# sailfish-team/sailfish

Measured on AMD Instinct MI355X. Metric: MLUPS (million lattice updates/s), D3Q19 BGK 512^3 per GPU, higher is better.
Workload: dtype f32; 1 GPU; D3Q19 BGK periodic box, 512x512x512 nodes per GPU, global 512x512x512 (fluid nodes only counted); access_pattern=AB, periodic=in-sweep wrap, decomposition=single subdomain, block_x=512, repeats=1

## Files before the change

sailfish_amd/csrc/slf_api.hip:

```cpp
#include <hip/hip_runtime.h>
#include <dlfcn.h>
#include <stdio.h>
#include <string.h>

#include <algorithm>
#include <string>
#include <vector>

#include "../../include/sailfish_hip.h"
#include "slf_kernels.h"
#include "slf_node.h"

#ifndef SLF_DEFAULT_VARIANT
#define SLF_DEFAULT_VARIANT 11
#endif

namespace {

thread_local std::string g_last_error;

int fail(int code, const std::string& msg) {
  g_last_error = msg;
  return code;
}

int hip_fail(hipError_t e, const char* what) {
  return fail(SLF_ERR_HIP, std::string(what) + ": " + hipGetErrorString(e));
}

#define SLF_HIP(call)                            \
  do {                                           \
    hipError_t _e = (call);                      \
    if (_e != hipSuccess) return hip_fail(_e, #call); \
  } while (0)

enum KernelKind {
  KK_COLLIDE_AND_PROPAGATE,
  KK_SET_INITIAL_CONDITIONS,
  KK_PBC,
  KK_PBC_SWAP,
  KK_MACRO_PBC,
  KK_COLLECT_SPARSE,
  KK_DISTRIBUTE_SPARSE,
  KK_COLLECT_BOX,
  KK_DISTRIBUTE_BOX,
  KK_COLLECT_FACE_SWAP,
  KK_DISTRIBUTE_FACE_SWAP,
  KK_COLLECT_MACRO_FACE,
  KK_DISTRIBUTE_MACRO_FACE,
  KK_COMPUTE_MACRO,
  KK_SC_MACRO,
  KK_SC_SWEEP0,
  KK_SC_SWEEP1,
  KK_SC_FUSED,
  KK_SC_INIT,
  KK_SCS_MACRO,
  KK_SCS_SWEEP,
  KK_RESIDENT,
};

}

struct slf_ctx {
  int device;
};
struct slf_stream {
  slf_ctx* ctx;
  hipStream_t s;
};
struct slf_event {
  slf_ctx* ctx;
  hipEvent_t e;
};
struct slf_graph {
  hipGraph_t graph;
  hipGraphExec_t exec;
};
struct slf_module {
  slf_ctx* ctx;
  slf::KernelSelector sel;
  slf::Geometry geo;
  slf::Physics phys;
  slf::ShanChen sc;
  int access_pattern;
  int block_x;
  void* node_params;
  uint32_t* status;
  void* xsend[2];
  void* xrecv[2];
  void* sc_send[3][2];
  void* sc_recv[3][2];
  slf::RowClasses rows;
  void* rows_mem;
  slf::SlotTable slots;
  void* slots_mem;
  int n_node_params, precision;
  void* stage[4];
  hipEvent_t stage_ev[4];
  size_t stage_bytes[4];
  int stage_next;
};
struct slf_kernel {
  slf_module* mod;
  KernelKind kind;
  std::vector<unsigned long long> ptrs;
  std::vector<long long> ints;
  int needs_iteration;
  uint32_t iteration;
  bool bound;
  bool sc_local_velocity;
  bool alpha_arg = false;
  int pair_rows = 0, pair_zc = 0;
  int pair_prefetch = 0;
};

static hipStream_t native(slf_stream* s) { return s ? s->s : (hipStream_t)0; }

static const slf::SlotTable* slot_table_for(slf_module* m, const void* nodes, hipStream_t s) {
  static const bool enabled = [] { const char* v = getenv("SLF_INDIRECT_SLOTS"); return !(v && atoi(v) == 0); }();
  if (!enabled || !nodes || !m->geo.indirect) return nullptr;
  if (m->slots.nodes == nodes) return &m->slots;
  if (m->geo.lat_ny > 65535 || m->geo.lat_nz > 65535) return nullptr;
  if (m->slots_mem) {
    hipFree(m->slots_mem);
    m->slots_mem = nullptr;
  }
  m->slots = slf::SlotTable{};
  const size_t n = m->geo.dist_size;
  char* mem = nullptr;
  if (hipMalloc((void**)&mem, 2 * n * sizeof(uint32_t) + 256) != hipSuccess) return nullptr;
  uint32_t* max_slot = (uint32_t*)(mem + 2 * n * sizeof(uint32_t));
  uint32_t h = 0;
  hipError_t e = hipMemsetAsync(mem, 0xFF, 2 * n * sizeof(uint32_t), s);
  if (e == hipSuccess) e = hipMemsetAsync(max_slot, 0, 256, s);
  if (e == hipSuccess) e = slf::launch_build_slot_table(m->geo, nodes, (uint32_t*)mem, (uint32_t*)mem + n, max_slot, s);
  if (e == hipSuccess) e = hipMemcpyAsync(&h, max_slot, sizeof(h), hipMemcpyDeviceToHost, s);
  if (e == hipSuccess) e = hipStreamSynchronize(s);
  if (e != hipSuccess) {
    hipFree(mem);
    return nullptr;
  }
  m->slots_mem = mem;
  m->slots.nodes = nodes;
  m->slots.slot_gi = (const uint32_t*)mem;
  m->slots.slot_yz = (const uint32_t*)mem + n;
  m->slots.n_slots = h + 1;
  return &m->slots;
}

extern "C" {

int slf_abi_version(void) { return SLF_ABI_VERSION; }

const char* slf_last_error(void) { return g_last_error.c_str(); }

int slf_device_count(int* count) {
  if (!count) return fail(SLF_ERR_INVALID, "count is NULL");
  hipError_t e = hipGetDeviceCount(count);
  if (e != hipSuccess) {
    *count = 0;
    return hip_fail(e, "hipGetDeviceCount");
  }
  return SLF_OK;
}

int slf_device_pci_bus_id(int device, char* out, size_t len) {
  if (!out || len < 13) return fail(SLF_ERR_INVALID, "buffer of at least 13 bytes needed");
  SLF_HIP(hipDeviceGetPCIBusId(out, (int)len, device));
  return SLF_OK;
}

int slf_ctx_create(int device, slf_ctx** out) {
  if (!out) return fail(SLF_ERR_INVALID, "out is NULL");
  int n = 0;
  SLF_HIP(hipGetDeviceCount(&n));
  if (device < 0 || device >= n) return fail(SLF_ERR_INVALID, "no such HIP device");
  SLF_HIP(hipSetDevice(device));
  slf_ctx* c = new slf_ctx;
  c->device = device;
  *out = c;
  return SLF_OK;
}

int slf_ctx_destroy(slf_ctx* ctx) {
  delete ctx;
  return SLF_OK;
}

int slf_ctx_sync(slf_ctx* ctx) {
  if (!ctx) return fail(SLF_ERR_INVALID, "ctx is NULL");
  SLF_HIP(hipSetDevice(ctx->device));
  SLF_HIP(hipDeviceSynchronize());
  return SLF_OK;
}

int slf_ctx_info(slf_ctx* ctx, char* name, size_t name_len, size_t* total_mem, int* cu_count, int* wavefront) {
  if (!ctx) return fail(SLF_ERR_INVALID, "ctx is NULL");
  hipDeviceProp_t prop;
  SLF_HIP(hipGetDeviceProperties(&prop, ctx->device));
  if (name && name_len) {
    snprintf(name, name_len, "%s (%s)", prop.name, prop.gcnArchName);
  }
  if (total_mem) *total_mem = prop.totalGlobalMem;
  if (cu_count) *cu_count = prop.multiProcessorCount;
  if (wavefront) *wavefront = prop.warpSize;
  return SLF_OK;
}

int slf_ctx_free_memory(slf_ctx* ctx, size_t* free_bytes) {
  if (!ctx || !free_bytes) return fail(SLF_ERR_INVALID, "NULL argument");
  SLF_HIP(hipSetDevice(ctx->device));
  size_t total = 0;
  SLF_HIP(hipMemGetInfo(free_bytes, &total));
  return SLF_OK;
}

int slf_malloc(slf_ctx* ctx, size_t bytes, void** dptr) {
  if (!ctx || !dptr) return fail(SLF_ERR_INVALID, "NULL argument");
  SLF_HIP(hipSetDevice(ctx->device));
  SLF_HIP(hipMalloc(dptr, bytes ? bytes : 1));
  return SLF_OK;
}

int slf_free(slf_ctx* ctx, void* dptr) {
  if (!ctx) return fail(SLF_ERR_INVALID, "ctx is NULL");
  if (dptr) SLF_HIP(hipFree(dptr));
  return SLF_OK;
}

int slf_memset(slf_ctx* ctx, void* dptr, int value, size_t bytes, slf_stream* stream) {
  if (!ctx || !dptr) return fail(SLF_ERR_INVALID, "NULL argument");
  SLF_HIP(hipMemsetAsync(dptr, value, bytes, native(stream)));
  if (!stream) SLF_HIP(hipStreamSynchronize(nullptr));
  return SLF_OK;
}

int slf_vmm_granularity(slf_ctx* ctx, size_t* bytes) {
  if (!ctx || !bytes) return fail(SLF_ERR_INVALID, "NULL argument");
  hipMemAllocationProp prop = {};
  prop.type = hipMemAllocationTypePinned;
  prop.location.type = hipMemLocationTypeDevice;
  prop.location.id = ctx->device;
  SLF_HIP(hipMemGetAllocationGranularity(bytes, &prop, hipMemAllocationGranularityRecommended));
  return SLF_OK;
}

int slf_vmm_reserve(slf_ctx* ctx, size_t bytes, void** va) {
  if (!ctx || !va) return fail(SLF_ERR_INVALID, "NULL argument");
  SLF_HIP(hipSetDevice(ctx->device));
  SLF_HIP(hipMemAddressReserve(va, bytes, 0, nullptr, 0));
  return SLF_OK;
}

int slf_vmm_release_range(slf_ctx* ctx, void* va, size_t bytes) {
  if (!ctx) return fail(SLF_ERR_INVALID, "ctx is NULL");
  SLF_HIP(hipMemAddressFree(va, bytes));
  return SLF_OK;
}

int slf_vmm_chunk_create(slf_ctx* ctx, size_t bytes, uint64_t* handle) {
  if (!ctx || !handle) return fail(SLF_ERR_INVALID, "NULL argument");
  SLF_HIP(hipSetDevice(ctx->device));
  hipMemAllocationProp prop = {};
  prop.type = hipMemAllocationTypePinned;
  prop.location.type = hipMemLocationTypeDevice;
  prop.location.id = ctx->device;
// ... 1260 lines not shown
      case 'i': k->ints.push_back(*(const int32_t*)argv[i]); break;
      default: return fail(SLF_ERR_INVALID, std::string("unsupported format char: ") + fmt[i]);
    }
  }
  const int dim = k->mod->geo.dim;
  size_t want_p = 0, want_i = 0;
  switch (k->kind) {
    case KK_COLLIDE_AND_PROPAGATE:
    case KK_COMPUTE_MACRO: want_p = 4 + dim; want_i = 1; break;
    case KK_SET_INITIAL_CONDITIONS: want_p = 3 + dim; want_i = 0; break;
    case KK_PBC:
    case KK_PBC_SWAP:
    case KK_MACRO_PBC: want_p = 1; want_i = 1; break;
    case KK_COLLECT_SPARSE:
    case KK_DISTRIBUTE_SPARSE: want_p = 3; want_i = 1; break;
    case KK_COLLECT_BOX:
    case KK_DISTRIBUTE_BOX:
      want_p = 2;
      want_i = (k->ints.size() == 8) ? 8 : 6;
      if (k->ints.size() == (dim == 3 ? 5u : 3u)) {
        want_i = k->ints.size();
        if (strcmp(fmt, dim == 3 ? "PiiiiiP" : "PiiiP")) return fail(SLF_ERR_INVALID, "reference form: the buffer is the last argument");
        if (k->mod->geo.indirect) return fail(SLF_ERR_UNSUPPORTED, "indirect addressing: halo through index lists");
      }
      break;
    case KK_COLLECT_FACE_SWAP:
    case KK_DISTRIBUTE_FACE_SWAP:
      want_p = 2; want_i = dim == 3 ? 5 : 3;
      if (strcmp(fmt, dim == 3 ? "PiiiiiP" : "PiiiP")) return fail(SLF_ERR_INVALID, "arguments: (dist, face, base_gx[, base_other], max_lx[, max_other], buffer)");
      break;
    case KK_COLLECT_MACRO_FACE:
    case KK_DISTRIBUTE_MACRO_FACE:
      want_p = 2; want_i = dim == 3 ? 5 : 3;
      if (strcmp(fmt, dim == 3 ? "PiiiiiP" : "PiiiP")) return fail(SLF_ERR_INVALID, "arguments: (field, [face,] base_gx, ..., buffer)");
      break;
    case KK_SC_MACRO:
    case KK_SC_SWEEP0:
    case KK_SC_SWEEP1: want_p = 5 + dim; want_i = 1; break;
    case KK_SC_FUSED: want_p = 7 + dim; want_i = 1; break;
    case KK_SC_INIT: want_p = 5 + dim; want_i = 0; break;
    case KK_SCS_MACRO: want_p = 3; want_i = 1; break;
    case KK_SCS_SWEEP: want_p = 4 + dim; want_i = 1; break;
    case KK_RESIDENT: want_p = 5; want_i = 5; break;
  }
  if (k->kind == KK_RESIDENT && k->ptrs.size() == 5 && k->ints.size() == 5) {
    const bool aa = k->mod->access_pattern == SLF_AA;
    const int steps = (int)k->ints[1], tx = (int)k->ints[2], ty = (int)k->ints[3], halo = (int)k->ints[4];
    if (!needs_iteration) return fail(SLF_ERR_INVALID, "CollideAndPropagateResident needs the iteration argument (its first step)");
    if (steps < 1 || tx < 1 || ty < 1 || halo < 1) return fail(SLF_ERR_INVALID, "steps, tile and halo must be positive");
    if (!k->ptrs[1] || !k->ptrs[3] || (!aa && (!k->ptrs[2] || !k->ptrs[4])))
      return fail(SLF_ERR_INVALID, "CollideAndPropagateResident: source and destination arrays (both copies of the two-copy pattern)");
    if (k->ptrs[1] == k->ptrs[3] || (!aa && k->ptrs[2] == k->ptrs[4]))
      return fail(SLF_ERR_INVALID, "CollideAndPropagateResident: source and destination must be different buffers");
    const int need = std::max(slf::resident_halo(aa, 0, steps), slf::resident_halo(aa, 1, steps));
    if (halo < need) return fail(SLF_ERR_INVALID, "CollideAndPropagateResident: halo too small for this many steps");
    const long long nw = (long long)(tx + 2 * halo) * (long long)(ty + 2 * halo);
    if (nw > 2 * 1024) return fail(SLF_ERR_INVALID, "CollideAndPropagateResident: window larger than 2048 nodes");
    const int q = 9;
    if (slf::resident_lds_bytes(q, k->mod->sel.precision, aa, tx + 2 * halo, ty + 2 * halo) + 4352 > 160 * 1024)
      return fail(SLF_ERR_INVALID, "CollideAndPropagateResident: window does not fit the 160 KiB of LDS");
  }
  if (k->mod->geo.indirect && (k->kind == KK_SC_FUSED || k->sc_local_velocity))
    return fail(SLF_ERR_UNSUPPORTED, "indirect addressing: the binary model runs the reference's pass and its two per-lattice sweeps");
  if (k->mod->geo.indirect && (k->kind == KK_COLLIDE_AND_PROPAGATE || k->kind == KK_COMPUTE_MACRO ||
                               k->kind == KK_SET_INITIAL_CONDITIONS || k->kind == KK_SC_MACRO ||
                               k->kind == KK_SC_SWEEP0 || k->kind == KK_SC_SWEEP1 || k->kind == KK_SC_INIT ||
                               k->kind == KK_SCS_MACRO || k->kind == KK_SCS_SWEEP))
    want_p += 1;
  k->alpha_arg = false;
  if (k->kind == KK_COLLIDE_AND_PROPAGATE && k->mod->sel.model == SLF_ELBM && k->ptrs.size() == want_p + 1 &&
      fmt[argc - 1] == 'P') {
    want_p += 1;
    k->alpha_arg = true;
  }
  if (k->ptrs.size() != want_p || k->ints.size() != want_i)
    return fail(SLF_ERR_INVALID, "argument list does not match the kernel's signature");
  k->pair_rows = k->pair_zc = 0;
  k->needs_iteration = needs_iteration;
  k->bound = true;
  if (k->kind == KK_COLLIDE_AND_PROPAGATE && k->mod->geo.indirect && !k->ptrs.empty() &&
      k->mod->phys.incompressible != SLF_DENSITY_ROUNDOFF && !k->mod->phys.regularized && !k->mod->phys.subgrid &&
      k->mod->sel.model != SLF_ELBM) {
    SLF_HIP(hipSetDevice(k->mod->ctx->device));
    slot_table_for(k->mod, (const void*)k->ptrs[0], (hipStream_t)0);
  }
  return SLF_OK;
}

int slf_kernel_set_iteration(slf_kernel* k, uint32_t iteration) {
  if (!k) return fail(SLF_ERR_INVALID, "kernel is NULL");
  k->iteration = iteration;
  return SLF_OK;
}

namespace {


int step_prop(const slf_kernel* k, slf::Prop* prop) {
  *prop = slf::PROP_AB;
  if (k->mod->access_pattern == SLF_AA) {
    if (!k->needs_iteration) return fail(SLF_ERR_INVALID, "AA kernels need the iteration argument");
    *prop = (k->iteration & 1u) ? slf::PROP_AA_ODD : slf::PROP_AA_EVEN;
  }
  return SLF_OK;
}

int sweep_region(const slf::Geometry& g, const slf_region* region, int* y0, int* y1, int* z0, int* z1) {
  *y0 = 1; *y1 = g.lat_ny - 1; *z0 = 1; *z1 = g.lat_nz - 1;
  if (g.dim == 2) { *z0 = 0; *z1 = 1; }
  if (region) {
    *y0 = region->y0; *y1 = region->y1;
    if (g.dim == 3) { *z0 = region->z0; *z1 = region->z1; }
    if (*y0 < 1 || *y1 > g.lat_ny - 1 || *y0 > *y1 || (g.dim == 3 && (*z0 < 1 || *z1 > g.lat_nz - 1 || *z0 > *z1)))
      return fail(SLF_ERR_INVALID, "region outside the real nodes of the subdomain");
  }
  return SLF_OK;
}

int sweep_common(const slf_kernel* k, slf::SweepArgs& a) {
  a.node_params = k->mod->node_params;
  a.status = k->mod->status;
  a.options = (uint32_t)k->ints[0];
  if (k->mod->sel.general && !a.map) return fail(SLF_ERR_INVALID, "node map is NULL but the module is not fluid_only");
  return SLF_OK;
}

void pair_args(const slf_kernel* k, slf::SweepArgs& a) {
  const slf_module* m = k->mod;
  const int b0 = m->geo.indirect ? 1 : 0;
  a.nodes = m->geo.indirect ? (const void*)k->ptrs[0] : nullptr;
  a.map = (const void*)k->ptrs[b0 + 0];
  a.dist_in = (void*)k->ptrs[b0 + 1];
  a.dist_out = (void*)k->ptrs[b0 + 2];
  a.node_params = m->node_params;
  a.status = m->status;
  a.options = (uint32_t)k->ints[0];
  for (int f = 0; f < 2; f++) {
    a.xsend[f] = m->xsend[f];
    a.xrecv[f] = m->xrecv[f];
  }
}

}

int slf_kernel_set_pair(slf_kernel* k, int rows_per_strip, int planes_per_chunk) {
  if (!k) return fail(SLF_ERR_INVALID, "kernel is NULL");
  if (k->kind != KK_COLLIDE_AND_PROPAGATE)
    return fail(SLF_ERR_UNSUPPORTED, "pair sweep: CollideAndPropagate kernels of single-fluid modules only");
  if (!k->bound) return fail(SLF_ERR_INVALID, "pair sweep: set the kernel arguments first (source and destination are checked)");
  if (rows_per_strip < 0 || planes_per_chunk < 0) return fail(SLF_ERR_INVALID, "pair sweep: negative strip / chunk size");
  const slf_module* m = k->mod;
  const int rows = rows_per_strip ? rows_per_strip : slf::pair_default_rows(m->geo);
  const int zc = planes_per_chunk ? planes_per_chunk : slf::pair_default_zchunk(m->geo);
  int prefetch = slf::pair_default_prefetch();
  if (const char* e = getenv("SLF_PAIR_PREFETCH")) {
    char* end = nullptr;
    const long v = strtol(e, &end, 10);
    if (*e) prefetch = (end && !*end && v >= 0 && v < 1000) ? (int)v : -1;
  }
  if (m->sc.enabled || m->sel.lattice != SLF_D3Q19 || k->alpha_arg)
    return fail(SLF_ERR_UNSUPPORTED, "pair sweep: D3Q19, single precision, BGK modules only");
  slf::SweepArgs a = {};
  pair_args(k, a);
  if (const char* why = slf::pair_refusal(m->sel, m->access_pattern == SLF_AB, m->geo, m->phys, a, rows, zc, prefetch))
    return fail(SLF_ERR_UNSUPPORTED, why);
  k->pair_rows = rows;
  k->pair_zc = zc;
  k->pair_prefetch = prefetch;
  return SLF_OK;
}

int slf_kernel_launch(slf_kernel* k, const slf_region* region, slf_stream* stream) {
  if (!k) return fail(SLF_ERR_INVALID, "kernel is NULL");
  if (!k->bound) return fail(SLF_ERR_INVALID, "kernel arguments not set");
  slf_module* m = k->mod;
  const slf::Geometry& g = m->geo;
  SLF_HIP(hipSetDevice(m->ctx->device));
  hipStream_t s = native(stream);
  hipError_t e = hipSuccess;
  switch (k->kind) {
    case KK_COLLIDE_AND_PROPAGATE:
    case KK_COMPUTE_MACRO: {
      if (k->pair_rows) {
        slf::SweepArgs pa = {};
        pair_args(k, pa);
        if (region) return fail(SLF_ERR_UNSUPPORTED, "pair sweep: whole-box launches only");
        if (!slf::launch_sweep_pair(m->sel, m->access_pattern == SLF_AB, g, m->phys, pa, k->pair_rows, k->pair_zc, k->pair_prefetch, s,
                                    &e)) {
          const char* why = slf::pair_refusal(m->sel, m->access_pattern == SLF_AB, g, m->phys, pa, k->pair_rows, k->pair_zc,
                                              k->pair_prefetch);
          return fail(SLF_ERR_UNSUPPORTED, why ? why : "pair sweep: no kernel for this strip size");
        }
        break;
      }
      slf::SweepArgs a = {};
      const int b0 = g.indirect ? 1 : 0;
      a.nodes = g.indirect ? (const void*)k->ptrs[0] : nullptr;
      a.map = (const void*)k->ptrs[b0 + 0];
      a.dist_in = (void*)k->ptrs[b0 + 1];
      a.dist_out = (void*)k->ptrs[b0 + 2];
      a.rho = (void*)k->ptrs[b0 + 3];
      a.phi = nullptr;
      a.v[0] = (void*)k->ptrs[b0 + 4];
      a.v[1] = (void*)k->ptrs[b0 + 5];
      a.v[2] = g.dim == 3 ? (void*)k->ptrs[b0 + 6] : nullptr;
      a.alpha = k->alpha_arg ? (void*)k->ptrs.back() : nullptr;
      for (int f = 0; f < 2; f++) {
        a.xsend[f] = m->xsend[f];
        a.xrecv[f] = m->xrecv[f];
      }
      a.rows = m->rows.map ? &m->rows : nullptr;
      if (int rc = sweep_common(k, a)) return rc;
      if (g.indirect && !a.nodes) return fail(SLF_ERR_INVALID, "indirect addressing: the nodes table is NULL");
      if (g.indirect && k->kind == KK_COLLIDE_AND_PROPAGATE && m->slots.nodes == a.nodes) a.slots = &m->slots;
      slf::Prop prop;
      if (int rc = step_prop(k, &prop)) return rc;
      if (k->kind == KK_COMPUTE_MACRO) {
        e = slf::launch_macro(m->sel, prop, g, m->phys, a, s);
        break;
      }
      int y0, y1, z0, z1;
      if (int rc = sweep_region(g, region, &y0, &y1, &z0, &z1)) return rc;
      e = slf::launch_sweep(m->sel, prop, g, m->phys, a, y0, y1, z0, z1, m->block_x, s);
      break;
    }
    case KK_SC_MACRO:
    case KK_SC_SWEEP0:
    case KK_SC_SWEEP1: {
      slf::SweepArgs a = {};
      const int b0 = g.indirect ? 1 : 0;
      a.nodes = g.indirect ? (const void*)k->ptrs[0] : nullptr;
      if (g.indirect && !a.nodes) return fail(SLF_ERR_INVALID, "indirect addressing: the nodes table is NULL");
      a.map = (const void*)k->ptrs[b0 + 0];
      a.dist_in = (void*)k->ptrs[b0 + 1];
      a.dist_out = (void*)k->ptrs[b0 + 2];
      a.rho = (void*)k->ptrs[b0 + 3];
      a.phi = (void*)k->ptrs[b0 + 4];
      a.v[0] = (void*)k->ptrs[b0 + 5];
      a.v[1] = (void*)k->ptrs[b0 + 6];
      a.v[2] = g.dim == 3 ? (void*)k->ptrs[b0 + 7] : nullptr;
      a.sc_local_velocity = k->sc_local_velocity;
      sc_planes_of(m, a);
      if (int rc = sweep_common(k, a)) return rc;
      slf::Prop prop;
      if (int rc = step_prop(k, &prop)) return rc;
      int y0, y1, z0, z1;
      if (int rc = sweep_region(g, region, &y0, &y1, &z0, &z1)) return rc;
      if (k->kind == KK_SC_MACRO) e = slf::launch_sc_macro(m->sel, prop, g, m->phys, m->sc, a, y0, y1, z0, z1, s);
      else e = slf::launch_sc_sweep(m->sel, k->kind == KK_SC_SWEEP0 ? 0 : 1, prop, g, m->phys, m->sc, a, y0, y1, z0, z1,
                                    m->block_x, s);
      break;
    }
    case KK_SC_FUSED: {
      slf::SweepArgs a = {};
      a.map = (const void*)k->ptrs[0];
      a.dist_in = (void*)k->ptrs[1];
      a.dist_out = (void*)k->ptrs[2];
      a.dist_in2 = (void*)k->ptrs[3];
      a.dist_out2 = (void*)k->ptrs[4];
      a.rho = (void*)k->ptrs[5];
      a.phi = (void*)k->ptrs[6];
      a.v[0] = (void*)k->ptrs[7];
      a.v[1] = (void*)k->ptrs[8];
      a.v[2] = g.dim == 3 ? (void*)k->ptrs[9] : nullptr;
      a.sc_local_velocity = k->sc_local_velocity;
      sc_planes_of(m, a);
      if (int rc = sweep_common(k, a)) return rc;
      slf::Prop prop;
      if (int rc = step_prop(k, &prop)) return rc;
      int y0, y1, z0, z1;
      if (int rc = sweep_region(g, region, &y0, &y1, &z0, &z1)) return rc;
      e = slf::launch_sc_fused(m->sel, prop, g, m->phys, m->sc, a, y0, y1, z0, z1, m->block_x, s);
      break;
    }
    case KK_RESIDENT: {
      slf::SweepArgs a = {};
      a.map = (const void*)k->ptrs[0];
      a.node_params = m->node_params;
      a.status = m->status;
      a.options = (uint32_t)k->ints[0] & ~1u;
      if (m->sel.general && !a.map) return fail(SLF_ERR_INVALID, "node map is NULL but the module is not fluid_only");
      const void* src[2] = {(const void*)k->ptrs[1], (const void*)k->ptrs[2]};
      void* dst[2] = {(void*)k->ptrs[3], (void*)k->ptrs[4]};
      e = slf::launch_resident(m->sel, m->access_pattern == SLF_AA, g, m->phys, a, src, dst, (int)k->iteration, (int)k->ints[1],
                               (int)k->ints[2], (int)k->ints[3], (int)k->ints[4], s);
      break;
    }
    case KK_SCS_MACRO:
    case KK_SCS_SWEEP: {
      slf::SweepArgs a = {};
      const int b0 = g.indirect ? 1 : 0;
      a.nodes = g.indirect ? (const void*)k->ptrs[0] : nullptr;
      if (g.indirect && !a.nodes) return fail(SLF_ERR_INVALID, "indirect addressing: the nodes table is NULL");
      a.map = (const void*)k->ptrs[b0 + 0];
      a.dist_in = (void*)k->ptrs[b0 + 1];
      a.phi = nullptr;
      if (k->kind == KK_SCS_MACRO) {
        a.dist_out = nullptr;
        a.rho = (void*)k->ptrs[b0 + 2];
        a.v[0] = a.v[1] = a.v[2] = nullptr;
      } else {
        a.dist_out = (void*)k->ptrs[b0 + 2];
        a.rho = (void*)k->ptrs[b0 + 3];
        a.v[0] = (void*)k->ptrs[b0 + 4];
        a.v[1] = (void*)k->ptrs[b0 + 5];
        a.v[2] = g.dim == 3 ? (void*)k->ptrs[b0 + 6] : nullptr;
      }
      sc_planes_of(m, a);
      if (int rc = sweep_common(k, a)) return rc;
      slf::Prop prop;
      if (int rc = step_prop(k, &prop)) return rc;
      if (k->kind == KK_SCS_MACRO) {
        e = slf::launch_scs_macro(m->sel, prop, g, m->phys, m->sc, a, s);
        break;
      }
      int y0, y1, z0, z1;
      if (int rc = sweep_region(g, region, &y0, &y1, &z0, &z1)) return rc;
      e = slf::launch_scs_sweep(m->sel, prop, g, m->phys, m->sc, a, y0, y1, z0, z1, m->block_x, s);
      break;
    }
    case KK_SC_INIT: {
      const int b0 = g.indirect ? 1 : 0;
      if (g.indirect && !k->ptrs[0]) return fail(SLF_ERR_INVALID, "indirect addressing: the nodes table is NULL");
      const void* v[3] = {(const void*)k->ptrs[b0 + 3], (const void*)k->ptrs[b0 + 4],
                          g.dim == 3 ? (const void*)k->ptrs[b0 + 5] : nullptr};
      e = slf::launch_sc_init(m->sel, g, m->phys, (void*)k->ptrs[b0 + 1], (void*)k->ptrs[b0 + 2],
                              (const void*)k->ptrs[b0 + 3 + g.dim], (const void*)k->ptrs[b0 + 4 + g.dim], v,
                              g.indirect ? (const void*)k->ptrs[0] : nullptr, s);
      break;
    }
    case KK_SET_INITIAL_CONDITIONS: {
      const int b0 = g.indirect ? 1 : 0;
      const void* v[3] = {(const void*)k->ptrs[b0 + 1], (const void*)k->ptrs[b0 + 2],
                          g.dim == 3 ? (const void*)k->ptrs[b0 + 3] : nullptr};
      if (g.indirect && !k->ptrs[0]) return fail(SLF_ERR_INVALID, "indirect addressing: the nodes table is NULL");
      e = slf::launch_init(m->sel, g, m->phys, (void*)k->ptrs[b0 + 0], (const void*)k->ptrs[b0 + 1 + g.dim], v,
                           g.indirect ? (const void*)k->ptrs[0] : nullptr, s);
      break;
    }
    case KK_PBC:
    case KK_PBC_SWAP:
      e = slf::launch_pbc(m->sel, g, (void*)k->ptrs[0], (int)k->ints[0], k->kind == KK_PBC_SWAP, s);
      break;
// ... 286 lines not shown
```

sailfish_amd/csrc/slf_kernels.h:

```cpp
#pragma once
#include <hip/hip_runtime.h>
#include <stdint.h>

namespace slf {

enum Prop : int { PROP_AB = 0, PROP_AA_EVEN = 1, PROP_AA_ODD = 2 };

struct Geometry {
  int dim;
  int lat_nx, lat_ny, lat_nz;
  int arr_nx, arr_ny, arr_nz;
  int arr_nxy;
  uint32_t dist_size;
  int wrap[3];
  int axis_mode[3];
  uint32_t type_mask;
  uint32_t param_shift;
  uint32_t param_mask;
  uint32_t orient_shift;
  unsigned long long type_lut;
  int use_link_tags;
  int variant;
  int indirect;
  int bc_level;
  int x_ghost_unused;
};

__host__ __device__ __forceinline__ int type_kind(unsigned long long type_lut, uint32_t dense_type) {
  return (int)((type_lut >> (4u * dense_type)) & 0xFull);
}
__host__ __device__ __forceinline__ int node_kind(unsigned long long type_lut, uint32_t type_mask, uint32_t code) {
  return type_kind(type_lut, code & type_mask);
}

struct Physics {
  double tau, visc;
  double accel[3];
  double mrt_rates[27];
  int incompressible;
  int has_force;
  int relaxation_enabled;
  int force_edm;
  int regularized, subgrid;
  double smagorinsky_const;
  int entropic_equilibrium;
  double entropy_tolerance, alpha_tolerance;
  uint32_t tms_mask;
};

struct ShanChen {
  int enabled;
  double tau_phi;
  double G[4];
  int potential;
  double accel1[3];
};

struct RowClasses;
struct SlotTable;

struct SweepArgs {
  const void* nodes;
  const void* map;
  void* dist_in;
  void* dist_out;
  void* dist_in2;
  void* dist_out2;
  void* rho;
  void* phi;
  void* v[3];
  const void* node_params;
  void* status;
  uint32_t options;
  bool sc_local_velocity;
  void* xsend[2];
  const void* xrecv[2];
  const SlotTable* slots;
  const RowClasses* rows;
  void* xsend2[2];
  const void* xrecv2[2];
  void* msend[2];
  const void* mrecv[2];
  void* alpha;
};

struct SlotTable {
  const void* nodes;
  const uint32_t* slot_gi;
  const uint32_t* slot_yz;
  uint32_t n_slots;
};

struct RowClasses {
  const void* map;
  const uint32_t* seg_class;
  const uint8_t* row_class;
  const uint32_t* bc_rows;
  int nseg;
  int n_rows, n_bc_rows;
  long long n_fluid_segments, n_segments;
};

struct KernelSelector {
  int lattice, model, precision;
  bool general;
};

hipError_t launch_sweep(const KernelSelector& sel, Prop prop, const Geometry& g, const Physics& ph,
                        const SweepArgs& a, int y0, int y1, int z0, int z1, int block_x, hipStream_t s);

hipError_t launch_init(const KernelSelector& sel, const Geometry& g, const Physics& ph, void* dist,
                       const void* rho, const void* const v[3], const void* nodes, hipStream_t s);

hipError_t launch_pbc(const KernelSelector& sel, const Geometry& g, void* dist, int axis, bool with_swap,
                      hipStream_t s);

hipError_t launch_macro_pbc(const KernelSelector& sel, const Geometry& g, void* field, int axis, hipStream_t s);

hipError_t launch_sparse(const KernelSelector& sel, bool collect, const unsigned long long* idx, void* dist, void* buffer,
                         int n, hipStream_t s);

hipError_t launch_box(const KernelSelector& sel, const Geometry& g, bool collect, void* dist, void* buffer,
                      const int* dirs, int nd, unsigned long long base, long long col_stride, int ncols, long long row_stride,
                      int nrows, long long buf_k_stride, long long buf_row_stride, bool deliver_all, hipStream_t s);

hipError_t launch_macro(const KernelSelector& sel, Prop prop, const Geometry& g, const Physics& ph,
                        const SweepArgs& a, hipStream_t s);

hipError_t launch_build_slot_table(const Geometry& g, const void* nodes, uint32_t* slot_gi, uint32_t* slot_yz,
                                   uint32_t* max_slot, hipStream_t s);
hipError_t launch_classify_rows(const Geometry& g, const void* map, uint32_t* seg_class, uint8_t* row_class,
                                uint32_t* bc_rows, uint32_t* counters, int nseg, hipStream_t s);

hipError_t launch_sc_macro(const KernelSelector& sel, Prop prop, const Geometry& g, const Physics& ph,
                           const ShanChen& sc, const SweepArgs& a, int y0, int y1, int z0, int z1, hipStream_t s);
hipError_t launch_sc_sweep(const KernelSelector& sel, int grid_idx, Prop prop, const Geometry& g, const Physics& ph,
                           const ShanChen& sc, const SweepArgs& a, int y0, int y1, int z0, int z1, int block_x,
                           hipStream_t s);
hipError_t launch_sc_fused(const KernelSelector& sel, Prop prop, const Geometry& g, const Physics& ph, const ShanChen& sc,
                           const SweepArgs& a, int y0, int y1, int z0, int z1, int block_x, hipStream_t s);
hipError_t launch_scs_macro(const KernelSelector& sel, Prop prop, const Geometry& g, const Physics& ph,
                            const ShanChen& sc, const SweepArgs& a, hipStream_t s);
hipError_t launch_scs_sweep(const KernelSelector& sel, Prop prop, const Geometry& g, const Physics& ph,
                            const ShanChen& sc, const SweepArgs& a, int y0, int y1, int z0, int z1, int block_x,
                            hipStream_t s);
hipError_t launch_sc_init(const KernelSelector& sel, const Geometry& g, const Physics& ph, void* dist1, void* dist2,
                          const void* rho, const void* phi, const void* const v[3], const void* nodes, hipStream_t s);

hipError_t launch_resident(const KernelSelector& sel, bool aa, const Geometry& g, const Physics& ph, const SweepArgs& a,
                           const void* const src[2], void* const dst[2], int it0, int steps, int tile_x, int tile_y, int halo,
                           hipStream_t s);
int resident_halo(bool aa, int it0, int steps);
size_t resident_lds_bytes(int q, int precision, bool aa, int win_x, int win_y);

const char* pair_refusal(const KernelSelector& sel, bool two_copy, const Geometry& g, const Physics& ph, const SweepArgs& a,
                         int rows, int zc, int prefetch);
bool launch_sweep_pair(const KernelSelector& sel, bool two_copy, const Geometry& g, const Physics& ph, const SweepArgs& a,
                       int rows, int zc, int prefetch, hipStream_t s, hipError_t* err);
int pair_default_rows(const Geometry& g);
int pair_default_zchunk(const Geometry& g);
int pair_default_prefetch();

constexpr int STATS_PROFILE_COUNT = 22;
struct StatsShape {
  int block, grid_x;
  int chunks, per_chunk;
  size_t workspace_doubles;
};
StatsShape stats_ke_shape(const Geometry& g);
StatsShape stats_profiles_shape(const Geometry& g, int axis);
hipError_t launch_stats_ke_enstrophy(const KernelSelector& sel, const Geometry& g, const void* map, const void* const v[3],
                                     void* v_sq, void* vort_sq, double* workspace, double* out2, hipStream_t s);
hipError_t launch_stats_profiles(const KernelSelector& sel, const Geometry& g, int axis, const void* const v[3],
                                 const void* rho, double* workspace, double* out, size_t out_stride, size_t offset,
                                 hipStream_t s);

}
```

sailfish_amd/csrc/slf_pair.hip:

```cpp
#include "slf_dispatch.h"
#include "slf_rowpush.h"

namespace slf {

namespace {

constexpr int PAIR_NT = 3;
constexpr int PAIR_NW = 8;

__device__ __forceinline__ int wrap1(int c, int n) {
  if (c < 1) c += n;
  if (c > n) c -= n;
  return c;
}

extern __shared__ float s_stage[];
#define SLF_LDS __attribute__((address_space(3)))

template <bool RAW>
__device__ __forceinline__ void pair_barrier() {
  if constexpr (RAW) {
    asm volatile("s_waitcnt lgkmcnt(0)" ::: "memory");
    __builtin_amdgcn_s_barrier();
    asm volatile("" ::: "memory");
  } else {
    __syncthreads();
  }
}

template <int MODEL, int TY, int PF>
__global__ void __launch_bounds__(512, TY == 2 ? 4 : 2) pair_row_kernel(const SweepParams<D3Q19, float> p, const int zc) {
  using L = D3Q19;
  static_assert(MODEL == 0, "BGK only");
  static_assert(TY % 2 == 0, "the push slots alternate by row");
  static_assert(PF == 0 || PF == 1, "ring depth");
  constexpr int NXD = count_x_dirs<L>();
  __shared__ float s_in_p[3][TY][PAIR_NW][NXD], s_in_m[3][TY][PAIR_NW][NXD];
  __shared__ float s_out_p[2][PAIR_NW][NXD], s_out_m[2][PAIR_NW][NXD];
  const Geometry& g = p.g;
  const int ny = g.lat_ny - 2, nz = g.lat_nz - 2;
  const int lane = (int)threadIdx.x & 63;
  const int w = sgpr((int)threadIdx.x >> 6);
  const int nwave = sgpr((int)blockDim.x >> 6);
  const int slot_p = sgpr(w == 0 ? nwave - 1 : w - 1);
  const int slot_m = sgpr(w == nwave - 1 ? 0 : w + 1);
  const int x = (int)threadIdx.x + 1;
  const uint32_t xb = (uint32_t)x * 4u;
  const int y0 = sgpr(1 + (int)blockIdx.y * TY);
  const int z0 = sgpr(1 + (int)blockIdx.z * zc);
  int zn = nz - (z0 - 1);
  if (zn > zc) zn = zc;
  zn = sgpr(zn);
  const size_t ds = g.dist_size;
  const AxisOff ox0 = {0, 0};
  const bool inc = p.cp.incompressible != 0;

  float P0[TY][L::Q], P1[TY][L::Q], P2[TY][L::Q];
  static_for<0, TY>([&](auto J) {
    static_for<0, L::Q>([&](auto I) { P0[J][I] = P1[J][I] = P2[J][I] = 0.0f; });
  });

  float* const stage_w = s_stage + sgpr(w * (L::Q * 64));
  const uint32_t stage_m0 = sgpr((uint32_t)(uintptr_t)(SLF_LDS float*)stage_w);
  const uint64_t dir_bytes = (uint64_t)ds * sizeof(float);
  const uint32_t dlo = sgpr((uint32_t)dir_bytes), dhi = sgpr((uint32_t)(dir_bytes >> 32));
  auto stage_row = [&](int gy, int gz) {
    const uint32_t row = sgpr((uint32_t)g.arr_nx * (uint32_t)gy + (uint32_t)g.arr_nxy * (uint32_t)gz);
    const uint64_t src = (uint64_t)(p.din + row);
    const uint32_t slo = sgpr((uint32_t)src), shi = sgpr((uint32_t)(src >> 32));
    uint32_t keep;
    static_assert(L::Q == 19 && (PAIR_NT & 1), "the statement below: 1 + 18 loads, nt");
    asm volatile(
        "s_mov_b32 %[keep], m0\n\t"
        "s_mov_b32 vcc_lo, %[slo]\n\t"
        "s_mov_b32 vcc_hi, %[shi]\n\t"
        "s_mov_b32 m0, %[lds]\n\t"
        "s_nop 0\n\t"
        "global_load_lds_dword %[xb], vcc nt\n\t"
        ".rept 18\n\t"
        "s_add_u32 m0, m0, 0x100\n\t"
        "s_add_u32 vcc_lo, vcc_lo, %[dlo]\n\t"
        "s_addc_u32 vcc_hi, vcc_hi, %[dhi]\n\t"
        "global_load_lds_dword %[xb], vcc nt\n\t"
        ".endr\n\t"
        "s_mov_b32 m0, %[keep]"
        : [keep] "=&s"(keep)
        : [slo] "s"(slo), [shi] "s"(shi), [lds] "s"(stage_m0), [dlo] "s"(dlo), [dhi] "s"(dhi), [xb] "v"(xb)
        : "vcc", "scc", "memory");
  };
  if constexpr (PF > 0) stage_row(sgpr(wrap1(y0 - 1, ny)), sgpr(wrap1(z0 - 1, nz)));

  int c0 = 0, c1 = 1, c2 = 2;
  for (int s = 0; s < zn + 2; s++) {
    const int gz = sgpr(wrap1(z0 - 1 + s, nz));
    const bool own_plane = s >= 1 && s <= zn;
    static_for<0, TY + 2>([&](auto RR) {
      constexpr int rr = (int)RR - 1;
      const int gy = sgpr(wrap1(y0 + rr, ny));
      float f[L::Q];
      if constexpr (PF > 0) {
        asm volatile("s_waitcnt vmcnt(0)" ::: "memory");
        static_for<0, L::Q>([&](auto I) { f[I] = stage_w[(int)I * 64 + lane]; });
        asm volatile("s_waitcnt lgkmcnt(0)" ::: "memory");
        if constexpr (rr < TY) stage_row(sgpr(wrap1(y0 + rr + 1, ny)), gz);
        else if (s + 1 < zn + 2) stage_row(sgpr(wrap1(y0 - 1, ny)), sgpr(wrap1(z0 + s, nz)));
      } else {
        const uint32_t row = sgpr((uint32_t)g.arr_nx * (uint32_t)gy + (uint32_t)g.arr_nxy * (uint32_t)gz);
        static_for<0, L::Q>([&](auto I) {
          f[I] = ldg<PAIR_NT>(at_byte(uniform_base(p.din + ds * (size_t)I + row), xb));
        });
      }
      float rho, v[3];
      macro_standard<L, float>(f, inc, rho, v);
      if constexpr (rr >= 0 && rr < TY) {
        if (own_plane) check_invalid<float>(p.status, p.options, rho, x, gy, gz);
      }
      if (p.relaxation_enabled) bgk_relax<L, float, false>(f, rho, v, p.cp);
      static_for<0, L::Q>([&](auto I) {
        constexpr int j = rr + L::ey(I);
        if constexpr (j >= 0 && j < TY) {
          if constexpr (L::ez(I) > 0) P2[j][I] = f[I];
          else if constexpr (L::ez(I) == 0) P1[j][I] = f[I];
          else P0[j][I] = f[I];
        }
      });
      if (lane == 63) {
        static_for<1, L::Q>([&](auto I) {
          constexpr int j = rr + L::ey(I);
          if constexpr (L::ex(I) > 0 && j >= 0 && j < TY)
            s_in_p[L::ez(I) > 0 ? c2 : (L::ez(I) == 0 ? c1 : c0)][j][w][x_dir_rank<L, I>()] = f[I];
        });
      }
      if (lane == 0) {
        static_for<1, L::Q>([&](auto I) {
          constexpr int j = rr + L::ey(I);
          if constexpr (L::ex(I) < 0 && j >= 0 && j < TY)
            s_in_m[L::ez(I) > 0 ? c2 : (L::ez(I) == 0 ? c1 : c0)][j][w][x_dir_rank<L, I>()] = f[I];
        });
      }
    });
    if (s >= 2) {
      const int gzb = sgpr(z0 + s - 2);
      AxisOff oz = axis_off(gzb, g.lat_nz, g.arr_nxy, 1);
      oz.p = sgpr(oz.p); oz.m = sgpr(oz.m);
      pair_barrier<(PF > 0)>();
      static_for<0, TY>([&](auto J) {
        constexpr int buf = (int)J & 1;
        float f[L::Q];
        {
          int kp = 0, km = 0;
          static_for<0, L::Q>([&](auto I) {
            if constexpr (L::ex(I) > 0) f[I] = lane_shift1<float, true>(s_in_p[c0][J][slot_p][kp++], P0[J][I]);
            else if constexpr (L::ex(I) < 0) f[I] = lane_shift1<float, false>(s_in_m[c0][J][slot_m][km++], P0[J][I]);
            else f[I] = P0[J][I];
          });
        }
        const int gy = sgpr(y0 + (int)J);
        float rho, v[3];
        macro_standard<L, float>(f, inc, rho, v);
        check_invalid<float>(p.status, p.options, rho, x, gy, gzb);
        if (p.relaxation_enabled) bgk_relax<L, float, false>(f, rho, v, p.cp);
        if (lane == 63) {
          int k = 0;
          static_for<1, L::Q>([&](auto I) { if constexpr (L::ex(I) > 0) s_out_p[buf][w][k++] = f[I]; });
        }
        if (lane == 0) {
          int k = 0;
          static_for<1, L::Q>([&](auto I) { if constexpr (L::ex(I) < 0) s_out_m[buf][w][k++] = f[I]; });
        }
        pair_barrier<(PF > 0)>();
        const uint32_t row = sgpr((uint32_t)g.arr_nx * (uint32_t)gy + (uint32_t)g.arr_nxy * (uint32_t)gzb);
        AxisOff oy = axis_off(gy, g.lat_ny, g.arr_nx, 1);
        oy.p = sgpr(oy.p); oy.m = sgpr(oy.m);
        int kp = 0, km = 0;
        static_for<0, L::Q>([&](auto I) {
          const int off = dir_offset<L, I>(ox0, oy, oz, true);
          const auto base = uniform_base(p.dout + ds * (size_t)I + (uint32_t)((int)row + off));
          float t = f[I];
          if constexpr (L::ex(I) > 0) t = lane_shift1<float, true>(s_out_p[buf][slot_p][kp++], f[I]);
          if constexpr (L::ex(I) < 0) t = lane_shift1<float, false>(s_out_m[buf][slot_m][km++], f[I]);
          stg<PAIR_NT>(at_byte(base, xb), t);
        });
      });
    }
    { const int t = c0; c0 = c1; c1 = c2; c2 = t; }
    static_for<0, TY>([&](auto J) {
      static_for<0, L::Q>([&](auto I) {
        if constexpr (L::ez(I) >= 0) P0[J][I] = P1[J][I];
        if constexpr (L::ez(I) > 0) P1[J][I] = P2[J][I];
      });
    });
  }
}

}

int pair_default_rows(const Geometry& g) { return (g.lat_ny - 2) % 4 == 0 ? 4 : 2; }
int pair_default_zchunk(const Geometry&) { return 64; }
int pair_default_prefetch() { return 1; }

const char* pair_refusal(const KernelSelector& sel, bool two_copy, const Geometry& g, const Physics& ph, const SweepArgs& a,
                         int rows, int zc, int prefetch) {
  if (sel.lattice != 1 || sel.precision != 4 || sel.model != 0) return "pair sweep: D3Q19, single precision, BGK modules only";
  if (!two_copy) return "pair sweep: the two-copy (AB) access pattern only";
  if (sel.general || a.map) return "pair sweep: modules without a node map only";
  if (g.indirect || a.nodes) return "pair sweep: direct addressing only";
  if (ph.has_force) return "pair sweep: body forces are not served";
  if (!(g.variant & 1) || (g.variant & 256)) return "pair sweep: the tuned kernels are switched off for this module";
  if (!g.wrap[0] || !g.wrap[1] || !g.wrap[2]) return "pair sweep: every axis must be wrapped inside the sweep";
  if (a.xsend[0] || a.xsend[1] || a.xrecv[0] || a.xrecv[1]) return "pair sweep: not with x-face buffers";
  const int nx = g.lat_nx - 2, ny = g.lat_ny - 2;
  if (nx % 64 != 0 || nx < 64 || nx > 64 * PAIR_NW) return "pair sweep: rows of 64 .. 512 nodes, a multiple of 64";
  if (rows != 2 && rows != 4) return "pair sweep: 2 or 4 rows per strip";
  if (ny % rows != 0) return "pair sweep: ny must be a multiple of the rows per strip";
  if (zc < 1) return "pair sweep: planes per chunk must be positive";
  if (prefetch != 0 && prefetch != 1) return "pair sweep: SLF_PAIR_PREFETCH is 0 (synchronous loads) or 1 (one row staged in LDS)";
  if (!a.dist_in || !a.dist_out) return "pair sweep: source or destination array is NULL";
  if (a.dist_in == a.dist_out) return "pair sweep: source and destination must be different arrays";
  if (a.options & 1u) return "pair sweep: macro field output is not served (options bit 0)";
  return nullptr;
}

bool launch_sweep_pair(const KernelSelector& sel, bool two_copy, const Geometry& g, const Physics& ph, const SweepArgs& a,
                       int rows, int zc, int prefetch, hipStream_t s, hipError_t* err) {
  if (pair_refusal(sel, two_copy, g, ph, a, rows, zc, prefetch)) return false;
  const SweepParams<D3Q19, float> p = make_params<D3Q19, float>(g, ph, a, 1, 1);
  const int nx = g.lat_nx - 2, ny = g.lat_ny - 2, nz = g.lat_nz - 2;
  if (zc > nz) zc = nz;
  dim3 block(nx, 1, 1);
  dim3 grid(1, ny / rows, (nz + zc - 1) / zc);
  const size_t lds = prefetch ? (size_t)(nx / 64) * D3Q19::Q * 64 * sizeof(float) : 0;
  const bool done = pick<int, 2, 4>(rows, [&](auto TY) {
    pick<int, 0, 1>(prefetch, [&](auto PF) {
      hipLaunchKernelGGL((pair_row_kernel<0, TY, PF>), grid, block, lds, s, p, zc);
    });
  });
  if (done) *err = hipGetLastError();
  return done;
}

}
```

Before: 56860 MLUPS.

## Remap pair-sweep strips across XCDs, alternate row march direction, drop nt loads

The pair sweep kernel now remaps blockIdx.y through an XCD-aware permutation (xcd_row with a shift chosen from the strip count), so consecutive y-strips land on the same XCD and neighbouring strips can share L2 halo rows. Odd strips walk their rows downward, so adjacent strips touch shared boundary rows at nearby times. The non-temporal hint on the row-staging global loads is removed by default, letting halo rows stay in cache. This targets repeated DRAM traffic for the halo rows read by neighbouring strips, at the cost of extra scalar index math and depends on the hardware's workgroup-to-XCD dispatch order matching the assumed mapping.

After: 61230 MLUPS (median of 6 runs). +7.7%, better.

```diff
diff --git a/sailfish_amd/csrc/slf_api.hip b/sailfish_amd/csrc/slf_api.hip
--- a/sailfish_amd/csrc/slf_api.hip
+++ b/sailfish_amd/csrc/slf_api.hip
@@ -112,6 +112,7 @@
   bool alpha_arg = false;
   int pair_rows = 0, pair_zc = 0;
   int pair_prefetch = 0;
+  int pair_xcd_log2 = 0, pair_march = 0;
 };
 
 static hipStream_t native(slf_stream* s) { return s ? s->s : (hipStream_t)0; }
@@ -1678,21 +1679,27 @@
   const slf_module* m = k->mod;
   const int rows = rows_per_strip ? rows_per_strip : slf::pair_default_rows(m->geo);
   const int zc = planes_per_chunk ? planes_per_chunk : slf::pair_default_zchunk(m->geo);
-  int prefetch = slf::pair_default_prefetch();
-  if (const char* e = getenv("SLF_PAIR_PREFETCH")) {
+  auto knob = [](const char* name, int dflt) {
+    const char* e = getenv(name);
+    if (!e || !*e) return dflt;
     char* end = nullptr;
     const long v = strtol(e, &end, 10);
-    if (*e) prefetch = (end && !*end && v >= 0 && v < 1000) ? (int)v : -1;
-  }
+    return (end && !*end && v >= 0 && v < 1000) ? (int)v : -1;
+  };
+  const int prefetch = knob("SLF_PAIR_PREFETCH", slf::pair_default_prefetch());
+  const int xcd_log2 = knob("SLF_PAIR_XCD_LOG2", slf::pair_default_xcd_log2());
+  const int march = knob("SLF_PAIR_MARCH", slf::pair_default_march());
   if (m->sc.enabled || m->sel.lattice != SLF_D3Q19 || k->alpha_arg)
     return fail(SLF_ERR_UNSUPPORTED, "pair sweep: D3Q19, single precision, BGK modules only");
   slf::SweepArgs a = {};
   pair_args(k, a);
-  if (const char* why = slf::pair_refusal(m->sel, m->access_pattern == SLF_AB, m->geo, m->phys, a, rows, zc, prefetch))
+  if (const char* why = slf::pair_refusal(m->sel, m->access_pattern == SLF_AB, m->geo, m->phys, a, rows, zc, prefetch, xcd_log2, march))
     return fail(SLF_ERR_UNSUPPORTED, why);
   k->pair_rows = rows;
   k->pair_zc = zc;
   k->pair_prefetch = prefetch;
+  k->pair_xcd_log2 = xcd_log2;
+  k->pair_march = march;
   return SLF_OK;
 }
 
@@ -1711,10 +1718,10 @@
         slf::SweepArgs pa = {};
         pair_args(k, pa);
         if (region) return fail(SLF_ERR_UNSUPPORTED, "pair sweep: whole-box launches only");
-        if (!slf::launch_sweep_pair(m->sel, m->access_pattern == SLF_AB, g, m->phys, pa, k->pair_rows, k->pair_zc, k->pair_prefetch, s,
-                                    &e)) {
+        if (!slf::launch_sweep_pair(m->sel, m->access_pattern == SLF_AB, g, m->phys, pa, k->pair_rows, k->pair_zc, k->pair_prefetch,
+                                    k->pair_xcd_log2, k->pair_march, s, &e)) {
           const char* why = slf::pair_refusal(m->sel, m->access_pattern == SLF_AB, g, m->phys, pa, k->pair_rows, k->pair_zc,
-                                              k->pair_prefetch);
+                                              k->pair_prefetch, k->pair_xcd_log2, k->pair_march);
           return fail(SLF_ERR_UNSUPPORTED, why ? why : "pair sweep: no kernel for this strip size");
         }
         break;
diff --git a/sailfish_amd/csrc/slf_kernels.h b/sailfish_amd/csrc/slf_kernels.h
--- a/sailfish_amd/csrc/slf_kernels.h
+++ b/sailfish_amd/csrc/slf_kernels.h
@@ -154,12 +154,15 @@
 size_t resident_lds_bytes(int q, int precision, bool aa, int win_x, int win_y);
 
 const char* pair_refusal(const KernelSelector& sel, bool two_copy, const Geometry& g, const Physics& ph, const SweepArgs& a,
-                         int rows, int zc, int prefetch);
+                         int rows, int zc, int prefetch, int xcd_log2, int march);
 bool launch_sweep_pair(const KernelSelector& sel, bool two_copy, const Geometry& g, const Physics& ph, const SweepArgs& a,
-                       int rows, int zc, int prefetch, hipStream_t s, hipError_t* err);
+                       int rows, int zc, int prefetch, int xcd_log2, int march, hipStream_t s, hipError_t* err);
 int pair_default_rows(const Geometry& g);
 int pair_default_zchunk(const Geometry& g);
 int pair_default_prefetch();
+int pair_default_xcd_log2();
+int pair_default_march();
+int pair_xcd_shift(int strips, int limit);
 
 constexpr int STATS_PROFILE_COUNT = 22;
 struct StatsShape {
diff --git a/sailfish_amd/csrc/slf_pair.hip b/sailfish_amd/csrc/slf_pair.hip
--- a/sailfish_amd/csrc/slf_pair.hip
+++ b/sailfish_amd/csrc/slf_pair.hip
@@ -6,6 +6,15 @@
 namespace {
 
 constexpr int PAIR_NT = 3;
+#ifndef SLF_PAIR_LOAD_NT
+#define SLF_PAIR_LOAD_NT 0
+#endif
+constexpr int PAIR_LOAD_NT = SLF_PAIR_LOAD_NT ? PAIR_NT : 0;
+#if SLF_PAIR_LOAD_NT
+#define SLF_PAIR_LOAD_HINT " nt"
+#else
+#define SLF_PAIR_LOAD_HINT ""
+#endif
 constexpr int PAIR_NW = 8;
 
 __device__ __forceinline__ int wrap1(int c, int n) {
@@ -29,7 +38,8 @@
 }
 
 template <int MODEL, int TY, int PF>
-__global__ void __launch_bounds__(512, TY == 2 ? 4 : 2) pair_row_kernel(const SweepParams<D3Q19, float> p, const int zc) {
+__global__ void __launch_bounds__(512, TY == 2 ? 4 : 2) pair_row_kernel(const SweepParams<D3Q19, float> p, const int zc,
+                                                                         const int xcd_shift, const int march) {
   using L = D3Q19;
   static_assert(MODEL == 0, "BGK only");
   static_assert(TY % 2 == 0, "the push slots alternate by row");
@@ -46,7 +56,9 @@
   const int slot_m = sgpr(w == nwave - 1 ? 0 : w + 1);
   const int x = (int)threadIdx.x + 1;
   const uint32_t xb = (uint32_t)x * 4u;
-  const int y0 = sgpr(1 + (int)blockIdx.y * TY);
+  const int strip = sgpr(xcd_row((int)blockIdx.y, xcd_shift));
+  const int y0 = sgpr(1 + strip * TY);
+  const bool down = sgpr((int)(march != 0 && (strip & 1) != 0)) != 0;
   const int z0 = sgpr(1 + (int)blockIdx.z * zc);
   int zn = nz - (z0 - 1);
   if (zn > zc) zn = zc;
@@ -69,76 +81,82 @@
     const uint64_t src = (uint64_t)(p.din + row);
     const uint32_t slo = sgpr((uint32_t)src), shi = sgpr((uint32_t)(src >> 32));
     uint32_t keep;
-    static_assert(L::Q == 19 && (PAIR_NT & 1), "the statement below: 1 + 18 loads, nt");
+    static_assert(L::Q == 19, "the statement below: 1 + 18 loads");
     asm volatile(
         "s_mov_b32 %[keep], m0\n\t"
         "s_mov_b32 vcc_lo, %[slo]\n\t"
         "s_mov_b32 vcc_hi, %[shi]\n\t"
         "s_mov_b32 m0, %[lds]\n\t"
         "s_nop 0\n\t"
-        "global_load_lds_dword %[xb], vcc nt\n\t"
+        "global_load_lds_dword %[xb], vcc" SLF_PAIR_LOAD_HINT "\n\t"
         ".rept 18\n\t"
         "s_add_u32 m0, m0, 0x100\n\t"
         "s_add_u32 vcc_lo, vcc_lo, %[dlo]\n\t"
         "s_addc_u32 vcc_hi, vcc_hi, %[dhi]\n\t"
-        "global_load_lds_dword %[xb], vcc nt\n\t"
+        "global_load_lds_dword %[xb], vcc" SLF_PAIR_LOAD_HINT "\n\t"
         ".endr\n\t"
         "s_mov_b32 m0, %[keep]"
         : [keep] "=&s"(keep)
         : [slo] "s"(slo), [shi] "s"(shi), [lds] "s"(stage_m0), [dlo] "s"(dlo), [dhi] "s"(dhi), [xb] "v"(xb)
         : "vcc", "scc", "memory");
   };
-  if constexpr (PF > 0) stage_row(sgpr(wrap1(y0 - 1, ny)), sgpr(wrap1(z0 - 1, nz)));
+  if constexpr (PF > 0) stage_row(sgpr(wrap1(down ? y0 + TY : y0 - 1, ny)), sgpr(wrap1(z0 - 1, nz)));
 
   int c0 = 0, c1 = 1, c2 = 2;
   for (int s = 0; s < zn + 2; s++) {
     const int gz = sgpr(wrap1(z0 - 1 + s, nz));
     const bool own_plane = s >= 1 && s <= zn;
-    static_for<0, TY + 2>([&](auto RR) {
-      constexpr int rr = (int)RR - 1;
-      const int gy = sgpr(wrap1(y0 + rr, ny));
-      float f[L::Q];
-      if constexpr (PF > 0) {
-        asm volatile("s_waitcnt vmcnt(0)" ::: "memory");
-        static_for<0, L::Q>([&](auto I) { f[I] = stage_w[(int)I * 64 + lane]; });
-        asm volatile("s_waitcnt lgkmcnt(0)" ::: "memory");
-        if constexpr (rr < TY) stage_row(sgpr(wrap1(y0 + rr + 1, ny)), gz);
-        else if (s + 1 < zn + 2) stage_row(sgpr(wrap1(y0 - 1, ny)), sgpr(wrap1(z0 + s, nz)));
-      } else {
-        const uint32_t row = sgpr((uint32_t)g.arr_nx * (uint32_t)gy + (uint32_t)g.arr_nxy * (uint32_t)gz);
+    auto phase_a = [&](auto DOWN) {
+      static_for<0, TY + 2>([&](auto M) {
+        constexpr bool dn = decltype(DOWN)::value;
+        constexpr int rr = dn ? TY - (int)M : (int)M - 1;
+        constexpr int step = dn ? -1 : 1, first = dn ? TY : -1;
+        const int gy = sgpr(wrap1(y0 + rr, ny));
+        float f[L::Q];
+        if constexpr (PF > 0) {
+          asm volatile("s_waitcnt vmcnt(0)" ::: "memory");
+          static_for<0, L::Q>([&](auto I) { f[I] = stage_w[(int)I * 64 + lane]; });
+          asm volatile("s_waitcnt lgkmcnt(0)" ::: "memory");
+          if constexpr ((int)M < TY + 1) stage_row(sgpr(wrap1(y0 + rr + step, ny)), gz);
+          else if (s + 1 < zn + 2) stage_row(sgpr(wrap1(y0 + first, ny)), sgpr(wrap1(z0 + s, nz)));
+        } else {
+          const uint32_t row = sgpr((uint32_t)g.arr_nx * (uint32_t)gy + (uint32_t)g.arr_nxy * (uint32_t)gz);
+          static_for<0, L::Q>([&](auto I) {
+            f[I] = ldg<PAIR_LOAD_NT>(at_byte(uniform_base(p.din + ds * (size_t)I + row), xb));
+          });
+        }
+        float rho, v[3];
+        macro_standard<L, float>(f, inc, rho, v);
+        if constexpr (rr >= 0 && rr < TY) {
+          if (own_plane) check_invalid<float>(p.status, p.options, rho, x, gy, gz);
+        }
+        if (p.relaxation_enabled) bgk_relax<L, float, false>(f, rho, v, p.cp);
         static_for<0, L::Q>([&](auto I) {
-          f[I] = ldg<PAIR_NT>(at_byte(uniform_base(p.din + ds * (size_t)I + row), xb));
+          constexpr int j = rr + L::ey(I);
+          if constexpr (j >= 0 && j < TY) {
+            if constexpr (L::ez(I) > 0) P2[j][I] = f[I];
+            else if constexpr (L::ez(I) == 0) P1[j][I] = f[I];
+            else P0[j][I] = f[I];
+          }
         });
-      }
-      float rho, v[3];
-      macro_standard<L, float>(f, inc, rho, v);
-      if constexpr (rr >= 0 && rr < TY) {
-        if (own_plane) check_invalid<float>(p.status, p.options, rho, x, gy, gz);
-      }
-      if (p.relaxation_enabled) bgk_relax<L, float, false>(f, rho, v, p.cp);
-      static_for<0, L::Q>([&](auto I) {
-        constexpr int j = rr + L::ey(I);
-        if constexpr (j >= 0 && j < TY) {
-          if constexpr (L::ez(I) > 0) P2[j][I] = f[I];
-          else if constexpr (L::ez(I) == 0) P1[j][I] = f[I];
-          else P0[j][I] = f[I];
+        if (lane == 63) {
+          static_for<1, L::Q>([&](auto I) {
+            constexpr int j = rr + L::ey(I);
+            if constexpr (L::ex(I) > 0 && j >= 0 && j < TY)
+              s_in_p[L::ez(I) > 0 ? c2 : (L::ez(I) == 0 ? c1 : c0)][j][w][x_dir_rank<L, I>()] = f[I];
+          });
+        }
+        if (lane == 0) {
+          static_for<1, L::Q>([&](auto I) {
+            constexpr int j = rr + L::ey(I);
+            if constexpr (L::ex(I) < 0 && j >= 0 && j < TY)
+              s_in_m[L::ez(I) > 0 ? c2 : (L::ez(I) == 0 ? c1 : c0)][j][w][x_dir_rank<L, I>()] = f[I];
+          });
         }
       });
-      if (lane == 63) {
-        static_for<1, L::Q>([&](auto I) {
-          constexpr int j = rr + L::ey(I);
-          if constexpr (L::ex(I) > 0 && j >= 0 && j < TY)
-            s_in_p[L::ez(I) > 0 ? c2 : (L::ez(I) == 0 ? c1 : c0)][j][w][x_dir_rank<L, I>()] = f[I];
-        });
-      }
-      if (lane == 0) {
-        static_for<1, L::Q>([&](auto I) {
-          constexpr int j = rr + L::ey(I);
-          if constexpr (L::ex(I) < 0 && j >= 0 && j < TY)
-            s_in_m[L::ez(I) > 0 ? c2 : (L::ez(I) == 0 ? c1 : c0)][j][w][x_dir_rank<L, I>()] = f[I];
-        });
-      }
-    });
+    };
+    if (down) phase_a(std::true_type{});
+    else phase_a(std::false_type{});
     if (s >= 2) {
       const int gzb = sgpr(z0 + s - 2);
       AxisOff oz = axis_off(gzb, g.lat_nz, g.arr_nxy, 1);
@@ -198,9 +216,17 @@
 int pair_default_rows(const Geometry& g) { return (g.lat_ny - 2) % 4 == 0 ? 4 : 2; }
 int pair_default_zchunk(const Geometry&) { return 64; }
 int pair_default_prefetch() { return 1; }
+int pair_default_xcd_log2() { return 5; }
+int pair_default_march() { return 1; }
+
+int pair_xcd_shift(int strips, int limit) {
+  int s = limit < 0 ? 0 : (limit > 8 ? 8 : limit);
+  while (s > 0 && (strips % (8 << s)) != 0) s--;
+  return s;
+}
 
 const char* pair_refusal(const KernelSelector& sel, bool two_copy, const Geometry& g, const Physics& ph, const SweepArgs& a,
-                         int rows, int zc, int prefetch) {
+                         int rows, int zc, int prefetch, int xcd_log2, int march) {
   if (sel.lattice != 1 || sel.precision != 4 || sel.model != 0) return "pair sweep: D3Q19, single precision, BGK modules only";
   if (!two_copy) return "pair sweep: the two-copy (AB) access pattern only";
   if (sel.general || a.map) return "pair sweep: modules without a node map only";
@@ -215,6 +241,9 @@
   if (ny % rows != 0) return "pair sweep: ny must be a multiple of the rows per strip";
   if (zc < 1) return "pair sweep: planes per chunk must be positive";
   if (prefetch != 0 && prefetch != 1) return "pair sweep: SLF_PAIR_PREFETCH is 0 (synchronous loads) or 1 (one row staged in LDS)";
+  if (xcd_log2 < 0 || xcd_log2 > 8)
+    return "pair sweep: SLF_PAIR_XCD_LOG2 is an integer in 0 .. 8 (consecutive strips per XCD = 1 << this at most; 0: off)";
+  if (march != 0 && march != 1) return "pair sweep: SLF_PAIR_MARCH is 0 (every strip walks its rows upwards) or 1 (odd strips downwards)";
   if (!a.dist_in || !a.dist_out) return "pair sweep: source or destination array is NULL";
   if (a.dist_in == a.dist_out) return "pair sweep: source and destination must be different arrays";
   if (a.options & 1u) return "pair sweep: macro field output is not served (options bit 0)";
@@ -222,17 +251,18 @@
 }
 
 bool launch_sweep_pair(const KernelSelector& sel, bool two_copy, const Geometry& g, const Physics& ph, const SweepArgs& a,
-                       int rows, int zc, int prefetch, hipStream_t s, hipError_t* err) {
-  if (pair_refusal(sel, two_copy, g, ph, a, rows, zc, prefetch)) return false;
+                       int rows, int zc, int prefetch, int xcd_log2, int march, hipStream_t s, hipError_t* err) {
+  if (pair_refusal(sel, two_copy, g, ph, a, rows, zc, prefetch, xcd_log2, march)) return false;
   const SweepParams<D3Q19, float> p = make_params<D3Q19, float>(g, ph, a, 1, 1);
   const int nx = g.lat_nx - 2, ny = g.lat_ny - 2, nz = g.lat_nz - 2;
   if (zc > nz) zc = nz;
   dim3 block(nx, 1, 1);
   dim3 grid(1, ny / rows, (nz + zc - 1) / zc);
+  const int shift = pair_xcd_shift((int)grid.y, xcd_log2);
   const size_t lds = prefetch ? (size_t)(nx / 64) * D3Q19::Q * 64 * sizeof(float) : 0;
   const bool done = pick<int, 2, 4>(rows, [&](auto TY) {
     pick<int, 0, 1>(prefetch, [&](auto PF) {
-      hipLaunchKernelGGL((pair_row_kernel<0, TY, PF>), grid, block, lds, s, p, zc);
+      hipLaunchKernelGGL((pair_row_kernel<0, TY, PF>), grid, block, lds, s, p, zc, shift, march);
     });
   });
   if (done) *err = hipGetLastError();
```
